# montekki/thaler-study

Hardware: AMD Instinct MI355X
Metric: field mul-adds/sec in sumcheck prover, n=28 vars (higher is better)
Workload: dtype u64

## Files before the change

thaler-study_amd/csrc/engine/abi_context.inc:

```


extern "C" int sc_field_from_modulus(uint64_t p, sc_field* out) {
  if (!out) return SC_ERR_ARG;
  sc::FieldParams fp;
  if (!sc::field_params_from_modulus(p, &fp)) return SC_ERR_ARG;
  out->p = fp.p;
  out->p_inv_neg = fp.p_inv_neg;
  out->r_mod_p = fp.r_mod_p;
  out->r2_mod_p = fp.r2_mod_p;
  return SC_OK;
}

static sc::FieldParams to_params(const sc_field* f) {
  sc::FieldParams fp;
  fp.p = f->p;
  fp.p_inv_neg = f->p_inv_neg;
  fp.r_mod_p = f->r_mod_p;
  fp.r2_mod_p = f->r2_mod_p;
  return fp;
}

extern "C" uint64_t sc_field_to_mont(const sc_field* f, uint64_t canonical) {
  HostField hf(to_params(f));
  return hf.mul(canonical % f->p, f->r2_mod_p);
// ... 70 lines not shown
  SC_CREATE_HIP(hipMemset(ctx->d_wg_tickets, 0, 64 * sizeof(unsigned)));
  SC_CREATE_HIP(hipHostGetDevicePointer((void**)&ctx->d_mailbox, ctx->h_mailbox, 0));
  SC_CREATE_HIP(hipHostMalloc(&ctx->h_tail, kTailSlots * kTailSlotWords * sizeof(u64), hipHostMallocMapped | hipHostMallocCoherent));
  memset(ctx->h_tail, 0, kTailSlots * kTailSlotWords * sizeof(u64));
  SC_CREATE_HIP(hipHostGetDevicePointer((void**)&ctx->d_tail, ctx->h_tail, 0));
  for (int i = kTailSlots - 1; i >= 0; --i) ctx->tail_free.push_back(i);
  SC_CREATE_HIP(hipDeviceSynchronize());
  for (int i = 0; i < sc_ctx::kTimerRing; ++i) {
    SC_CREATE_HIP(hipEventCreate(&ctx->kt_ev[i][0]));
    SC_CREATE_HIP(hipEventCreate(&ctx->kt_ev[i][1]));
  }
#undef SC_CREATE_HIP
  *out = ctx;
  return SC_OK;
}

extern "C" int sc_ctx_destroy(sc_ctx* ctx) {
  if (!ctx) return SC_OK;
  if (is_multi(ctx)) return multi_destroy(ctx);
  (void)hipSetDevice(ctx->device);
  if (ctx->stream) (void)sync_stream(ctx);
  if (ctx->comm && g_rccl.CommDestroy) g_rccl.CommDestroy(ctx->comm);
  for (int q = 0; q < sc::kMaxPeers; ++q)
    if (ctx->peer_ipc_opened[q] && ctx->peer_base[q]) (void)hipIpcCloseMemHandle(ctx->peer_base[q]);
  if (ctx->peer_region) (void)hipFree(ctx->peer_region);
  for (auto& kv : ctx->pool_free) (void)hipFree(kv.second);
  for (auto& kv : ctx->pool_live) (void)hipFree(kv.first);
  if (ctx->d_partials) (void)hipFree(ctx->d_partials);
  if (ctx->d_wg_partials) (void)hipFree(ctx->d_wg_partials);
  if (ctx->d_wg_groups) (void)hipFree(ctx->d_wg_groups);
  if (ctx->d_wg_tickets) (void)hipFree(ctx->d_wg_tickets);
  if (ctx->d_gram_rows) (void)hipFree(ctx->d_gram_rows);
  if (ctx->d_sums) (void)hipFree(ctx->d_sums);
  if (ctx->h_sums) (void)hipHostFree(ctx->h_sums);
  if (ctx->h_mailbox) (void)hipHostFree(ctx->h_mailbox);
  if (ctx->h_tail) (void)hipHostFree(ctx->h_tail);
  if (ctx->h_points) (void)hipHostFree(ctx->h_points);
  if (ctx->d_points) (void)hipFree(ctx->d_points);
  for (u64* tw : ctx->d_rs_twiddles)
    if (tw) (void)hipFree(tw);
  for (u64* tw : ctx->d_rs_twist)
    if (tw) (void)hipFree(tw);
  if (ctx->d_xc_inv) (void)hipFree(ctx->d_xc_inv);
  if (ctx->h_batch_desc) (void)hipHostFree(ctx->h_batch_desc);
  if (ctx->h_batch) (void)hipHostFree(ctx->h_batch);
  if (ctx->d_ticket) (void)hipFree(ctx->d_ticket);
  for (int i = 0; i < sc_ctx::kTimerRing; ++i)
    for (int k = 0; k < 2; ++k)
      if (ctx->kt_ev[i][k]) (void)hipEventDestroy(ctx->kt_ev[i][k]);
  if (ctx->stream) (void)hipStreamDestroy(ctx->stream);
  delete ctx;
  return SC_OK;
}

extern "C" const char* sc_last_error(const sc_ctx* ctx) {
  return ctx ? ctx->err.c_str() : g_create_error.c_str();
}

static int prewarm(sc_ctx* ctx, size_t num_vars);

enum : unsigned { kOptBool = 1, kOptOff = 2, kOptPeer = 4 };
struct OptionSpec {
  const char* name;
  int sc_ctx::*member;
  int64_t lo, hi;
  unsigned flags;
};
const OptionSpec kOptions[] = {
    {"vars_per_pass", &sc_ctx::vars_per_pass, 1, 2, 0},
    {"first_pass_vars", &sc_ctx::first_pass_vars, 0, 4, 0},
    {"grid_pass", &sc_ctx::grid_pass, 0, 1, kOptBool},
    {"grid_log", &sc_ctx::grid_log, 0, 26, 0},
    {"grid_max_vars", &sc_ctx::grid_max_vars, 1, sc::kGridMaxVars, 0},
    {"grid_sharded", &sc_ctx::grid_sharded, 0, 1, kOptBool},
    {"grid_blocks", &sc_ctx::grid_blocks, 0, kWgMaxBlocks, 0},
    {"fold_dma", &sc_ctx::fold_dma, 0, 1, kOptBool},
    {"pipe32", &sc_ctx::pipe32, 0, 1, kOptBool},
    {"pipe32_log", &sc_ctx::pipe32_log, 11, 40, 0},
    {"gram_log", &sc_ctx::gram_log, 14, 40, kOptOff},
    {"wfold_log", &sc_ctx::wfold_log, 12, 40, kOptOff},
    {"wfold_min_log", &sc_ctx::wfold_min_log, 12, 40, 0},
    {"wfold5_min_log", &sc_ctx::wfold5_min_log, 12, 40, 0},
    {"wfold_always", &sc_ctx::wfold_always, 0, 1, kOptBool},
    {"matmul_path", &sc_ctx::matmul_path, 0, 2, 0},
    {"host_tail_log", &sc_ctx::host_tail_log, 0, kTailLogMax, 0},
    {"gp_host_log", &sc_ctx::gp_host_log, 0, sc::kGpHostLogMax, 0},
    {"gp_tree_lv", &sc_ctx::gp_tree_lv, 1, 3, 0},
    {"fr_host_log", &sc_ctx::fr_host_log, 0, sc::kFrHostLogMax, 0},
    {"fr_tree_lv", &sc_ctx::fr_tree_lv, 1, sc::kFrTreeLvMax, 0},
    {"tail_log", &sc_ctx::tail_log, 0, 40, 0},
    {"max_blocks", &sc_ctx::max_blocks, 1, INT64_MAX, 0},
    {"time_kernels", &sc_ctx::time_kernels, 0, 1, kOptBool},
    {"use_mailbox", &sc_ctx::use_mailbox, 0, 1, kOptBool},
    {"nt_load_log", &sc_ctx::nt_load_log, INT64_MIN, INT64_MAX, 0},
    {"nt_store_log", &sc_ctx::nt_store_log, INT64_MIN, INT64_MAX, 0},
    {"pool_contiguous", &sc_ctx::pool_contiguous, 0, 1, kOptBool},
    {"dbg_fold_grab", &sc_ctx::dbg_fold_grab, 0, 16, 0},
    {"rccl_timeout_ms", &sc_ctx::rccl_timeout_ms, 1, 3600000, 0},
    {"arena_log", &sc_ctx::arena_log, 4, 26, kOptPeer},
    {"peer_spin_ms", &sc_ctx::peer_spin_ms, 1, 600000, kOptPeer},
    {"peer_connect_ms", &sc_ctx::peer_connect_ms, 1, 3600000, kOptPeer},
    {"dbg_delay_ms", &sc_ctx::dbg_delay_ms, 0, 10000, kOptPeer},
    {"dbg_skip_tag", &sc_ctx::dbg_skip_tag, 0, 1, kOptBool | kOptPeer},
};
static const OptionSpec* find_option(const char* key) {
  for (const OptionSpec& o : kOptions)
    if (strcmp(o.name, key) == 0) return &o;
  return nullptr;
}

extern "C" int sc_ctx_set_option(sc_ctx* ctx, const char* key, int64_t value) {
  if (!ctx || !key) return SC_ERR_ARG;
  const std::string k(key);
  if (k == "prewarm") return value < 0 ? fail(ctx, SC_ERR_ARG, "prewarm: num_vars must be >= 0") : prewarm(ctx, (size_t)value);
  if (is_multi(ctx)) SC_TRY(multi_set_option(ctx, key, value));
  if (k == "stat_reset") {
    ctx->stat_wait_ns = ctx->stat_launch_ns = 0;
    ctx->pool_peak_words = ctx->pool_live_words;
    return SC_OK;
  }
  const OptionSpec* o = find_option(key);
  if (!o) return fail(ctx, SC_ERR_ARG, "unknown option '%s'", key);
  if (o->member == &sc_ctx::max_blocks && (value < 1 || value > (int64_t)ctx->partial_rows))
    return fail(ctx, SC_ERR_ARG, "max_blocks must be 1..%zu", ctx->partial_rows);
  if (!(o->flags & kOptBool) && (value < o->lo || value > o->hi) && !((o->flags & kOptOff) && value == 0))
    return fail(ctx, SC_ERR_ARG, "%s must be %s%lld..%lld", key, (o->flags & kOptOff) ? "0 (never) or " : "", (long long)o->lo, (long long)o->hi);
  if (o->member == &sc_ctx::arena_log && ctx->peer_region) return fail(ctx, SC_ERR_STATE, "arena_log must be set before sc_ctx_comm_peer_export");
  ctx->*o->member = (o->flags & kOptBool) ? (value ? 1 : 0) : (int)value;
  return SC_OK;
}

static int64_t pool_stat(const sc_ctx* ctx, size_t (*of)(const sc_ctx*)) {
  if (!is_multi(ctx)) return (int64_t)of(ctx);
  int64_t sum = 0;
  for (const sc_ctx* sub : ctx->subs) sum += (int64_t)of(sub);
  return sum;
}

extern "C" int sc_ctx_get_option(const sc_ctx* ctx, const char* key, int64_t* value) {
  if (!ctx || !key || !value) return SC_ERR_ARG;
  const std::string k(key);
  if (k == "stat_wait_ns") *value = (int64_t)(is_multi(ctx) ? ctx->subs[0]->stat_wait_ns : ctx->stat_wait_ns);
  else if (k == "stat_launch_ns") *value = (int64_t)(is_multi(ctx) ? ctx->subs[0]->stat_launch_ns : ctx->stat_launch_ns);
  else if (k == "stat_pool_live_blocks") *value = pool_stat(ctx, [](const sc_ctx* c) { return c->pool_live.size(); });
  else if (k == "stat_pool_live_words") *value = pool_stat(ctx, [](const sc_ctx* c) { return c->pool_live_words; });
  else if (k == "stat_pool_peak_words") *value = pool_stat(ctx, [](const sc_ctx* c) { return c->pool_peak_words; });
  else if (k == "transport") *value = (int64_t)ctx->transport;
  else if (k == "n_devices") *value = is_multi(ctx) ? (int64_t)ctx->subs.size() : 1;
  else if (k == "comm_nranks") {
    int n = ctx->world;
    if (ctx->transport == Transport::kRccl) {
      n = 0;
      if (!g_rccl.CommCount || !ctx->comm || g_rccl.CommCount(ctx->comm, &n) != ncclSuccess)
        return fail(ctx, SC_ERR_RCCL, "ncclCommCount failed");
    }
    *value = n;
  } else if (const OptionSpec* o = find_option(key)) {
    *value = ctx->*o->member;
  } else {
    return fail(ctx, SC_ERR_ARG, "unknown option '%s'", key);
  }
  return SC_OK;
}

extern "C" int sc_ctx_synchronize(sc_ctx* ctx) {
  if (!ctx) return SC_ERR_ARG;
// ... 46 lines not shown
```

thaler-study_amd/csrc/engine/launch.inc:

```

namespace {


#define SC_DISPATCH_FIELD(ctx, F, f, ...)      \
  do {                                         \
    if ((ctx)->gold) {                         \
      typedef sc::GoldilocksMont F;            \
      F f((ctx)->fp);                          \
      __VA_ARGS__;                             \
    } else {                                   \
      typedef sc::MontGeneric F;               \
      F f((ctx)->fp);                          \
      __VA_ARGS__;                             \
    }                                          \
  } while (0)

template <int V>
using IntC = std::integral_constant<int, V>;
template <int... Vs, class Fn>
void with_const(int v, Fn&& fn) {
  (void)((v == Vs && (fn(IntC<Vs>{}), true)) || ...);
}
template <class Fn>
void with_bool(bool b, Fn&& fn) {
// ... 203 lines not shown
    hipLaunchKernelGGL(sc::mailbox_copy_wide_kernel, dim3(1), dim3(sc::kBlock), 0, ctx->stream, (const u64*)ctx->d_sums, 2 * cells,
                       ctx->d_mailbox, wo.seq);
    SC_HIP(ctx, hipGetLastError());
  }
  ctx->mailbox_seq += 1;
  return SC_OK;
}

bool in_tail(const sc_ctx* ctx, const u64* p) { return p && ctx->d_tail && p >= ctx->d_tail && p < ctx->d_tail + kTailSlots * kTailSlotWords; }

int launch_pass(sc_ctx* ctx, int kf, int ks, const u64* A, const u64* B, u64* A2, u64* B2, const u64* r,
                int log_in, bool across_ranks, bool* from_mailbox) {
  if (kf < 0 || kf > 4 || ks < 1 || ks > 3 || (ks == 3 && kf != 0) || (kf == 4 && (ks != 2 || log_in < 12)) || log_in < kf + ks)
    return fail(ctx, SC_ERR_ARG, "launch_pass: kf=%d ks=%d log_in=%d", kf, ks, log_in);
  const sc::FoldW fw = make_weights<sc::FoldW>(ctx, r, kf);
  size_t n_units = (size_t)1 << (log_in - kf - ks);
  const bool pipe32 = kf == 3 && ks == 2 && ctx->pipe32 && n_units % sc::kWave == 0 && log_in >= ctx->pipe32_log;
  const size_t bs = (size_t)sc::pass_block_threads(kf, ks, pipe32 ? 4 : 0);
  int grid = (int)std::min<size_t>(std::max<size_t>((n_units + bs - 1) / bs, 1), (size_t)ctx->max_blocks);
  grid = std::min(grid, pipe32 ? pipe32_resident_blocks(ctx) : pass_resident_blocks(ctx, kf, ks));
  if (kf > 0 && in_tail(ctx, A2) && (grid != 1 || ((size_t)1 << (log_in - kf)) > (size_t)sc::kWave))
    return fail(ctx, SC_ERR_STATE, "launch_pass: a pass_kernel launch of %d blocks would hand 2^%d-entry tables to the host with plain stores", grid,
                log_in - kf);
  const sc::PassOut out = next_pass_out(ctx, across_ranks, challenge_digest(r, kf, ks, log_in), from_mailbox);
  SC_TRY(timer_begin(ctx, SC_KIND_PASS, kf, ks, log_in, (u64)16 << log_in, kf > 0 ? (u64)16 << (log_in - kf) : 0));
  SC_DISPATCH_FIELD(ctx, F, f, launch_pass_t<F>(ctx, f, kf, ks, A, B, A2, B2, fw, n_units, grid, log_in, out, pipe32));
  SC_TRY(commit_pass_out(ctx, out, grid));
  SC_TRY(timer_end(ctx));
  return SC_OK;
}

int wait_mailbox(sc_ctx* ctx, u64 seq);

int check_exchange(sc_ctx* ctx, const char* what) {
  const u64 err = __atomic_load_n(ctx->h_mailbox + sc::kMailboxErr, __ATOMIC_ACQUIRE);
  if (err == 0) return SC_OK;
  if (err & (u64)sc::kXchgTimeout) {
    poison(ctx);
    return fail(ctx, SC_ERR_RCCL, "peer exchange: a rank's %s did not arrive within %d ms (rank %d waited for rank %d at tag %u; that rank's "
                "slot held tag ..%04x)", what, ctx->peer_spin_ms, ctx->rank, (int)((err >> 8) & 0xFF), ctx->xchg_tag, (unsigned)((err >> 16) & 0x3FFF));
  }
  return fail(ctx, SC_ERR_STATE, "the ranks of this sharded prover were given different challenges");
}

int launch_grid_pass(sc_ctx* ctx, int kf, int ks, const u64* A, const u64* B, u64* A2, u64* B2, const u64* r, int log_in, bool across_ranks) {
  if (kf < 0 || kf > sc::kGridMaxVars || ks < 1 || ks > sc::kGridMaxVars || log_in < kf + ks)
    return fail(ctx, SC_ERR_ARG, "launch_grid_pass: kf=%d ks=%d log_in=%d", kf, ks, log_in);
  if (!ctx->use_mailbox) return fail(ctx, SC_ERR_STATE, "launch_grid_pass needs the host mailbox");
  const sc::GridW gw = make_weights<sc::GridW>(ctx, r, kf);
  const size_t n_out = (size_t)1 << (log_in - kf);
  const int resident = std::min(resident_grid(ctx, ctx->gold ? kernel_ptr(&sc::wgrid_pass_kernel<sc::GoldilocksMont, 5, false>)
                                                             : kernel_ptr(&sc::wgrid_pass_kernel<sc::MontGeneric, 5, false>),
                                              sc::kBlock, 2 * ctx->num_cus),
                                kWgMaxBlocks);
  constexpr size_t kWaves = sc::kBlock / sc::kWave;
  const size_t n_iter = (n_out + sc::kWgEntries - 1) / sc::kWgEntries;
  const size_t cap = ctx->grid_blocks > 0 ? (size_t)std::min(ctx->grid_blocks, resident) : (size_t)resident;
  const int grid = (int)std::max<size_t>(1, std::min<size_t>((n_iter + kWaves - 1) / kWaves, cap));
  const sc::WgOut wo = next_wide_out(ctx, across_ranks, challenge_digest(r, kf, ks, log_in), true, in_tail(ctx, A2));
  SC_TRY(timer_begin(ctx, SC_KIND_GRID_PASS, kf, ks, log_in, (u64)16 << log_in, kf > 0 ? (u64)16 << (log_in - kf) : 0));
  const bool pf = (kf == 0 || kf == 2) && n_iter > (size_t)grid * kWaves;
  SC_DISPATCH_FIELD(ctx, F, f, with_bool(pf, [&](auto PF) {
    with_const<1, 2, 3, 4, 5>(ks, [&](auto KS) {
      hipLaunchKernelGGL((sc::wgrid_pass_kernel<F, KS, PF>), dim3(grid), dim3(sc::kBlock), 0, ctx->stream, f, A, B, A2, B2, gw, kf, n_out, wo);
    });
  }));
  return commit_wide_out(ctx, wo, pow3(ks));
}
bool wfold_has(int kf, int ks) { return (kf == 4 && ks == 5) || (kf == 5 && ks >= 3 && ks <= 5); }
int wfold_resident_blocks(sc_ctx* ctx) {
  const void* fn = ctx->gold ? kernel_ptr(&sc::wfold_pass_kernel<sc::GoldilocksMont, 4, 5, true>)
                             : kernel_ptr(&sc::wfold_pass_kernel<sc::MontGeneric, 4, 5, true>);
  return std::min(resident_grid(ctx, fn, sc::kWfThreads, ctx->num_cus), kWgMaxBlocks);
}
int launch_wfold_pass(sc_ctx* ctx, int kf, int ks, const u64* A, const u64* B, u64* A2, u64* B2, const u64* r, int log_in, bool across_ranks) {
  if (log_in < 12 || !A2 || !B2 || !wfold_has(kf, ks)) return fail(ctx, SC_ERR_ARG, "launch_wfold_pass: kf=%d ks=%d log_in=%d", kf, ks, log_in);
  if (!ctx->use_mailbox) return fail(ctx, SC_ERR_STATE, "launch_wfold_pass needs the host mailbox");
  const sc::FoldW fw = make_weights<sc::FoldW>(ctx, r, 4);
  const u64 r_top = kf == 5 ? r[4] : 0;
  const size_t n_tiles = (size_t)1 << (log_in - 12);
  const int grid = (int)std::max<size_t>(1, std::min<size_t>(std::min<size_t>(n_tiles, (size_t)wfold_resident_blocks(ctx)), (size_t)ctx->max_blocks));
  const sc::WgOut wo = next_wide_out(ctx, across_ranks, challenge_digest(r, kf, ks, log_in) ^ 0x77666f6cu, true, false);
  SC_TRY(timer_begin(ctx, SC_KIND_WFOLD_PASS, kf, ks, log_in, (u64)16 << log_in, (u64)16 << (log_in - kf)));
  SC_DISPATCH_FIELD(ctx, F, f, with_bool(log_in >= ctx->nt_load_log, [&](auto NT) {
    auto go = [&](auto KF, auto KS) {
      hipLaunchKernelGGL((sc::wfold_pass_kernel<F, KF, KS, NT>), dim3(grid), dim3(sc::kWfThreads), 0, ctx->stream, f, A, B, A2, B2, fw, r_top, n_tiles, wo);
    };
    if (kf == 4) go(IntC<4>{}, IntC<5>{});
    else with_const<3, 4, 5>(ks, [&](auto KS) { go(IntC<5>{}, KS); });
  }));
  return commit_wide_out(ctx, wo, pow3(ks));
}

constexpr int kGramK = 4;
constexpr int kGramMaxBlocks = 1024;
int gram_workspace(sc_ctx* ctx) {
  if (ctx->d_gram_rows) return SC_OK;
  const size_t bytes = (size_t)kGramMaxBlocks * sc::kGramRowWords * sizeof(u64) + 64;
  u64* p = nullptr;
  SC_HIP(ctx, hipMalloc(&p, bytes));
  hipError_t e = hipMemsetAsync(p, 0, bytes, ctx->stream);
  const int lds = sc::kGramStages * sc::kGramStageBytes;
  const void* fns[4] = {reinterpret_cast<const void*>(&sc::gram_pass_kernel<sc::GoldilocksMont, kGramK, true>),
                        reinterpret_cast<const void*>(&sc::gram_pass_kernel<sc::GoldilocksMont, kGramK, false>),
                        reinterpret_cast<const void*>(&sc::gram_pass_kernel<sc::MontGeneric, kGramK, true>),
                        reinterpret_cast<const void*>(&sc::gram_pass_kernel<sc::MontGeneric, kGramK, false>)};
  for (int i = 0; i < 4 && e == hipSuccess; ++i) e = hipFuncSetAttribute(fns[i], hipFuncAttributeMaxDynamicSharedMemorySize, lds);
  if (e != hipSuccess) {
    (void)hipFree(p);
    SC_HIP(ctx, e);
  }
  ctx->d_gram_rows = p;
  return SC_OK;
}
int launch_gram_pass(sc_ctx* ctx, const u64* A, const u64* B, int log_in, bool across_ranks) {
  typedef sc::GramGeo<kGramK> G;
  if (!ctx->use_mailbox) return fail(ctx, SC_ERR_STATE, "launch_gram_pass needs the host mailbox");
  const size_t len = (size_t)1 << log_in;
  if (len < (size_t)G::kEntriesPerStep * sc::kGramStages) return fail(ctx, SC_ERR_ARG, "launch_gram_pass: 2^%d entries are too few", log_in);
  const size_t n_steps = len / G::kEntriesPerStep;
  size_t blocks = 1;
  while (blocks * 2 <= (size_t)std::min(std::min(ctx->num_cus, ctx->max_blocks), kGramMaxBlocks)) blocks *= 2;
  size_t n_partials = std::min(blocks, n_steps / sc::kGramStages);
  while (n_steps / n_partials > (size_t)G::kMaxSteps) n_partials *= 2;
  const size_t spp = n_steps / n_partials;
  const int grid = (int)std::min(blocks, n_partials);
  SC_TRY(gram_workspace(ctx));
  const sc::WgOut wo = next_wide_out(ctx, across_ranks, challenge_digest(nullptr, 0, kGramK, log_in) ^ 0x6772616du, false, false);
  unsigned* ticket = reinterpret_cast<unsigned*>(ctx->d_gram_rows + (size_t)kGramMaxBlocks * sc::kGramRowWords);
  SC_TRY(timer_begin(ctx, SC_KIND_GRAM_PASS, 0, kGramK, log_in, (u64)16 << log_in, (u64)grid * sc::kGramRowWords * sizeof(u64)));
  const unsigned char* a8 = reinterpret_cast<const unsigned char*>(A);
  const unsigned char* b8 = reinterpret_cast<const unsigned char*>(B);
  const int lds = sc::kGramStages * sc::kGramStageBytes;
  SC_DISPATCH_FIELD(ctx, F, f, with_bool(log_in >= ctx->nt_load_log, [&](auto NT) {
    hipLaunchKernelGGL((sc::gram_pass_kernel<F, kGramK, NT>), dim3(grid), dim3(sc::kGramThreads), lds, ctx->stream, f, a8, b8,
                       (unsigned)n_partials, (unsigned)spp, ctx->d_gram_rows, ticket, wo);
  }));
  return commit_wide_out(ctx, wo, pow3(kGramK));
}

int collect_grid(sc_ctx* ctx, int ks, bool across_ranks, u64* out) {
  SC_TRY(wait_mailbox(ctx, ctx->mailbox_seq));
  const int cells = pow3(ks);
  const u64* wide = ctx->h_mailbox + sc::kMailboxWide;
  if (!across_ranks) {
    for (int c = 0; c < cells; ++c) out[c] = wide[c];
    return SC_OK;
  }
  HostField hf(ctx->fp);
  if (ctx->transport == Transport::kHost) {
    std::vector<u64> limbs(2 * (size_t)cells);
    for (int c = 0; c < cells; ++c) {
      limbs[2 * c] = wide[c] & 0xFFFFFFFFull;
      limbs[2 * c + 1] = wide[c] >> 32;
    }
    if (ctx->host_allreduce(ctx->host_user, limbs.data(), limbs.size()) != 0)
      return fail(ctx, SC_ERR_RCCL, "host all-reduce callback failed");
    for (int c = 0; c < cells; ++c) out[c] = hf.recombine(limbs[2 * c], limbs[2 * c + 1]);
    return SC_OK;
  }
  if (ctx->transport == Transport::kPeer) SC_TRY(check_exchange(ctx, "sums"));
  for (int c = 0; c < cells; ++c) out[c] = hf.recombine(wide[2 * c], wide[2 * c + 1]);
  return SC_OK;
}

int rank_pass(sc_ctx* ctx, int kf, const u64* A, const u64* B, u64* A2, u64* B2, const u64* r, u64* out) {
  if (ctx->transport != Transport::kPeer || !ctx->use_mailbox || kf < 0 || kf > sc::kGridMaxVars || ctx->log_world < 1 || ctx->log_world > 3)
    return fail(ctx, SC_ERR_STATE, "rank_pass: needs the peer transport, the mailbox and 2..8 ranks");
  const sc::GridW gw = make_weights<sc::GridW>(ctx, r, kf);
  const sc::WgOut wo = next_wide_out(ctx, true, challenge_digest(r, kf, ctx->log_world, kf) ^ 0x72616e6bu, true, false);
  SC_TRY(timer_begin(ctx, SC_KIND_GRID_PASS, kf, ctx->log_world, kf, (u64)16 << kf, (u64)16 << ctx->log_world));
  SC_DISPATCH_FIELD(ctx, F, f,
// ... 10 lines not shown
```

thaler-study_amd/csrc/kernels/grid_pass.hpp:

```cpp
#pragma once

namespace sc {

constexpr int kGridChunk = 256;
constexpr int kGridMaxVars = 5;
constexpr int kGridMaxCells = 243;
constexpr int kMailboxWide = 64;
constexpr int kMailboxWords = kMailboxWide + 512;
constexpr int kWgEntries = 32;
constexpr int kWgGroupBlocks = 32;
struct GridW {
  u64 w[1 << kGridMaxVars];
};
struct WgOut {
  u64* partials;
  u64* group_rows;
  unsigned* tickets;
  u64* mailbox;
  u64 seq;
  u64* limbs_dev;
  PeerX px;
  int host_out = 0;
};
template <class F, int KF>
// ... 279 lines not shown
    return;
  }
  if (tid < CELLS) __hip_atomic_store(out.mailbox + kMailboxWide + tid, total, __ATOMIC_RELAXED, __HIP_MEMORY_SCOPE_SYSTEM);
  asm volatile("s_waitcnt vmcnt(0)" ::: "memory");
  __syncthreads();
  if (tid == 0) __hip_atomic_store(out.mailbox + kMailboxSeq, out.seq, __ATOMIC_RELEASE, __HIP_MEMORY_SCOPE_SYSTEM);
}

template <class F, int KS>
__device__ __forceinline__ void wgrid_finish(const F& f, u64 total, const WgOut& out) {
  constexpr int kPow3[6] = {1, 3, 9, 27, 81, 243};
  constexpr int cells = kPow3[KS];
  __shared__ int lds_flag;
  const int tid = threadIdx.x;
  if (gridDim.x > 1) {
    const int n_blocks = gridDim.x, group = blockIdx.x / kWgGroupBlocks, n_groups = (n_blocks + kWgGroupBlocks - 1) / kWgGroupBlocks;
    const int group_size = min(kWgGroupBlocks, n_blocks - group * kWgGroupBlocks);
    if (tid < cells)
      __hip_atomic_store(out.partials + (size_t)blockIdx.x * kGridChunk + tid, total, __ATOMIC_RELAXED, __HIP_MEMORY_SCOPE_AGENT);
    asm volatile("s_waitcnt vmcnt(0)" ::: "memory");
    __syncthreads();
    if (tid == 0) {
      const unsigned t = __hip_atomic_fetch_add(out.tickets + 1 + group, 1u, __ATOMIC_RELAXED, __HIP_MEMORY_SCOPE_AGENT);
      const int last = (t == (unsigned)group_size - 1) ? 1 : 0;
      if (last) {
        __builtin_amdgcn_fence(__ATOMIC_ACQUIRE, "agent");
        asm volatile("s_waitcnt vmcnt(0)" ::: "memory");
      }
      lds_flag = last;
    }
    __syncthreads();
    if (!lds_flag) return;
    total = 0;
    if (tid < cells) {
      u64 x[kWgGroupBlocks];
#pragma unroll
      for (int q = 0; q < kWgGroupBlocks; ++q)
        x[q] = (q < group_size) ? __hip_atomic_load(out.partials + (size_t)(group * kWgGroupBlocks + q) * kGridChunk + tid, __ATOMIC_RELAXED,
                                                    __HIP_MEMORY_SCOPE_AGENT)
                                : 0;
#pragma unroll
      for (int q = 0; q < kWgGroupBlocks; ++q) total = f.add(total, x[q]);
    }
    if (n_groups > 1) {
      __syncthreads();
      if (tid < cells)
        __hip_atomic_store(out.group_rows + (size_t)group * kGridChunk + tid, total, __ATOMIC_RELAXED, __HIP_MEMORY_SCOPE_AGENT);
      asm volatile("s_waitcnt vmcnt(0)" ::: "memory");
      __syncthreads();
      if (tid == 0) {
        const unsigned t = __hip_atomic_fetch_add(out.tickets, 1u, __ATOMIC_RELAXED, __HIP_MEMORY_SCOPE_AGENT);
        const int last = (t == (unsigned)n_groups - 1) ? 1 : 0;
        if (last) {
          __builtin_amdgcn_fence(__ATOMIC_ACQUIRE, "agent");
          asm volatile("s_waitcnt vmcnt(0)" ::: "memory");
        }
        lds_flag = last;
      }
      __syncthreads();
      if (!lds_flag) return;
      total = 0;
      if (tid < cells) {
        u64 x[kWgGroupBlocks];
#pragma unroll
        for (int q = 0; q < kWgGroupBlocks; ++q)
          x[q] = (q < n_groups) ? __hip_atomic_load(out.group_rows + (size_t)q * kGridChunk + tid, __ATOMIC_RELAXED, __HIP_MEMORY_SCOPE_AGENT) : 0;
#pragma unroll
        for (int q = 0; q < kWgGroupBlocks; ++q) total = f.add(total, x[q]);
      }
    }
    if (tid <= n_groups) __hip_atomic_store(out.tickets + tid, 0u, __ATOMIC_RELAXED, __HIP_MEMORY_SCOPE_AGENT);
  }
  publish_cells<cells>(out, total);
}

template <class F, int KS, bool PF>
__global__ void __launch_bounds__(kBlock)
wgrid_pass_kernel(F f, const u64* __restrict__ A, const u64* __restrict__ B, u64* __restrict__ A2, u64* __restrict__ B2,
                  GridW gw, int kf, size_t n_out, WgOut out) {
  const u64 total = wgrid_body<F, KS, PF>(f, A, B, A2, B2, gw, kf, n_out, out.host_out != 0);
  wgrid_finish<F, KS>(f, total, out);
}

constexpr int kWfThreads = 512;
template <class F, int KF, int KS, bool NT>
__global__ void __launch_bounds__(kWfThreads)
wfold_pass_kernel(F f, const u64* __restrict__ A, const u64* __restrict__ B, u64* __restrict__ A2, u64* __restrict__ B2, FoldW fw,
                  u64 r_top, size_t n_tiles, WgOut out) {
  static_assert(KF == 4 || KF == 5, "four or five pending challenges");
  static_assert(KS >= 1 && KS <= 5, "one to five rounds");
  constexpr int OUT = 4, NPS = 8, NP = 32;
  constexpr int OUTS = kWave >> (KF - 4);
  constexpr int TILE_OUT = OUT * OUTS;
  constexpr int NPO = TILE_OUT / (2 * kWave);
  constexpr int kWaves = kWfThreads / kWave;
  constexpr int kPow3[6] = {1, 3, 9, 27, 81, 243};
  constexpr int cells = kPow3[KS], G = 1 << KS, gpi = kWgEntries >> KS, pairs = gpi * cells;
  constexpr int kRegionWords = 1024 + 512 + 512;
  __shared__ u64 lds_all[kWaves * kRegionWords];
  __shared__ int cell_of[kWgEntries], suffix_of[kWgEntries];
  __shared__ unsigned lds_next;
  typedef __attribute__((address_space(3))) u64 lds_u64;
  const int tid = threadIdx.x, lane = tid & (kWave - 1), wave = tid / kWave;
  if (tid < kWgEntries) {
    int c = 0, u = 0, p3 = 1;
    for (int m = 0; m < KS; ++m) {
      c += ((tid >> (KS - 1 - m)) & 1) * p3;
      u += ((tid >> m) & 1) * p3;
      p3 *= 3;
    }
    cell_of[tid] = c;
    suffix_of[tid] = u;
  }
  if (tid == 0) lds_next = 0;
  __syncthreads();
  ull2* const reg = reinterpret_cast<ull2*>(lds_all + (size_t)wave * kRegionWords);
  u64* const xchg = lds_all + (size_t)wave * kRegionWords + 1024;
  u64* const ef = xchg + 512;
  const int tbl = lane >> 5, ent = lane & (kWgEntries - 1);
  const int slot = tbl * kGridChunk + (ent >> KS) * cells + cell_of[ent & (G - 1)];
  unsigned step[KS][3];
#pragma clang loop unroll(full)
  for (int j = 0; j < KS; ++j) {
    const int low = KS - 1 - j, pj = kPow3[j], stride = kPow3[low], items = (gpi * pj) << low;
    const unsigned inv = (1u << 20) / (unsigned)pj + 1u;
#pragma clang loop unroll(full)
    for (int q = 0; q < 3; ++q) {
      const int idx = lane + kWave * q;
      unsigned d = 0;
      if (idx < 2 * items) {
        const int tb = idx >= items ? 1 : 0, id = idx - tb * items;
        const int sfx = id & ((1 << low) - 1), t = id >> low;
        const int g = (int)(((unsigned)t * inv) >> 20), pp = t - g * pj;
        d = 0x80000000u | (unsigned)(size_t)(lds_u64*)(ef + tb * kGridChunk + g * cells + pp * 3 * stride + suffix_of[sfx]);
      }
      step[j][q] = d;
    }
  }
  typename F::Acc acc[4];
#pragma unroll
  for (int k = 0; k < 4; ++k) f.acc_zero(acc[k]);

  const ull2* __restrict__ Ap = reinterpret_cast<const ull2*>(A);
  const ull2* __restrict__ Bp = reinterpret_cast<const ull2*>(B);
  ull2* __restrict__ A2p = reinterpret_cast<ull2*>(A2);
  ull2* __restrict__ B2p = reinterpret_cast<ull2*>(B2);
  const int rot = wave & 3;
  auto next_tile = [&]() -> size_t {
    unsigned c = 0;
    if (lane == 0) c = __hip_atomic_fetch_add(&lds_next, 1u, __ATOMIC_RELAXED, __HIP_MEMORY_SCOPE_WORKGROUP);
    return (size_t)__builtin_amdgcn_readfirstlane(c) * gridDim.x + blockIdx.x;
  };
  auto load_sub = [&](const ull2* __restrict__ T, size_t tile, int o, ull2 (&p)[NPS]) {
    const ull2* src = T + tile * kWave * NP + (size_t)o * NPS * kWave + lane;
#pragma unroll
    for (int k = 0; k < NPS; ++k) p[k] = ld16<NT>(src + k * kWave);
  };
  auto stash = [&](const ull2 (&p)[NPS]) {
#pragma unroll
    for (int k = 0; k < NPS; ++k) reg[swz_slot<NPS>(64 * k + lane)] = p[k];
  };
  auto fold16 = [&]() -> u64 {
    typename F::Acc3 sacc;
    f.acc3_zero(sacc);
#pragma unroll
    for (int m = 0; m < NPS; ++m) {
      const ull2 x = reg[swz_slot<NPS>(NPS * lane + m)];
      f.acc3_mac(sacc, x.x, fw.w[2 * m]);
      f.acc3_mac(sacc, x.y, fw.w[2 * m + 1]);
    }
    const u64 h = f.acc3_get(sacc);
    if constexpr (KF == 5) {
      const u64 hn = __shfl_xor(h, 1);
      return f.add(h, f.mul(r_top, f.sub(hn, h)));
    } else {
      return h;
    }
  };
  auto put = [&](u64* dst, int o, u64 x) {
    if constexpr (KF == 5) {
      if ((lane & 1) == 0) dst[OUTS * o + (lane >> 1)] = x;
    } else {
      dst[OUTS * o + lane] = x;
    }
  };
  auto grid_group = [&](int grp) {
    ef[slot] = xchg[kWave * OUT * tbl + kWgEntries * grp + ent];
    wave_lds_sync();
#pragma clang loop unroll(full)
    for (int j = 0; j < KS; ++j) {
      const int st = kPow3[KS - 1 - j];
#pragma clang loop unroll(full)
      for (int q = 0; q < 3; ++q) {
        if (2 * ((gpi * kPow3[j]) << (KS - 1 - j)) > kWave * q) {
          const unsigned d = step[j][q];
          if (d != 0) {
            lds_u64* const x = (lds_u64*)(size_t)(d & 0x7FFFFFFFu);
            x[2 * st] = f.sub(x[st], x[0]);
          }
        }
      }
      wave_lds_sync();
    }
#pragma unroll
    for (int k = 0; k < 4; ++k) {
      const int p = lane + kWave * k;
      if (p < pairs) f.acc_mac(acc[k], ef[p], ef[kGridChunk + p]);
    }
    wave_lds_sync();
  };
  ull2 pa[NPS], pb[NPS];
  size_t tile = next_tile();
  if (tile < n_tiles) {
    load_sub(Ap, tile, rot, pa);
    load_sub(Bp, tile, rot, pb);
  }
  while (tile < n_tiles) {
    const size_t next = next_tile();
#pragma unroll
    for (int i = 0; i < OUT; ++i) {
      const int o = (i + rot) & 3, no = (i + 1 + rot) & 3;
      stash(pa);
      wave_lds_sync();
      if (i + 1 < OUT) load_sub(Ap, tile, no, pa);
      else if (next < n_tiles) load_sub(Ap, next, no, pa);
      const u64 xa = fold16();
      wave_lds_sync();
      stash(pb);
      wave_lds_sync();
      if (i + 1 < OUT) load_sub(Bp, tile, no, pb);
      else if (next < n_tiles) load_sub(Bp, next, no, pb);
      const u64 xb = fold16();
      put(xchg, o, xa);
      put(xchg + kWave * OUT, o, xb);
      wave_lds_sync();
#pragma unroll 1
      for (int g = 0; g < OUTS / kWgEntries; ++g) grid_group(o * (OUTS / kWgEntries) + g);
    }
    {
      const ull2* xo = reinterpret_cast<const ull2*>(xchg);
      const size_t o0 = tile * kWave * NPO;
#pragma unroll
      for (int k = 0; k < NPO; ++k) {
        const size_t q = o0 + (size_t)k * kWave + lane;
        st16<false>(A2p + q, xo[kWave * k + lane]);
        st16<false>(B2p + q, xo[kWave * OUT / 2 + kWave * k + lane]);
      }
    }
    wave_lds_sync();
    if (wave == 0 && blockIdx.x < 8) asm volatile("buffer_wbl2 sc1" ::: "memory");
    tile = next;
  }
  __syncthreads();
  u64* const red = lds_all;
#pragma unroll
  for (int k = 0; k < 4; ++k) {
    const int p = lane + kWave * k;
    red[wave * kGridChunk + p] = (p < pairs) ? f.acc_get(acc[k]) : 0;
  }
  __syncthreads();
  u64 total = 0;
  if (tid < cells) {
    for (int w = 0; w < kWaves; ++w)
      for (int g = 0; g < gpi; ++g) total = f.add(total, red[w * kGridChunk + g * cells + tid]);
  }
  wgrid_finish<F, KS>(f, total, out);
}

template <class F>
__global__ void __launch_bounds__(kBlock)
rank_pass_kernel(F f, const u64* __restrict__ A, const u64* __restrict__ B, u64* __restrict__ A2, u64* __restrict__ B2, GridW gw, int kf,
                 WgOut out) {
  const PeerX& px = out.px;
  __shared__ u64 ta[kMaxPeers], tb[kMaxPeers];
  __shared__ int worst;
  const int tid = threadIdx.x;
  const size_t par = (size_t)(px.tag & 1u) * kMaxPeers * kInboxWords;
  int err = 0;
  if (tid == 0) worst = 0;
  if (tid < 2) {
    const u64* __restrict__ src = tid ? B : A;
    const int fan = 1 << kf;
    u64 v = 0;
    for (int c = 0; c < fan; ++c) v = f.add(v, f.mul(src[c], gw.w[c]));
    const ull2 pair = {((u64)px.tag << 32) | (v & 0xFFFFFFFFull), ((u64)px.tag << 32) | (v >> 32)};
    const size_t mine = par + (size_t)px.rank * kInboxWords + kInboxWide + 2 * (size_t)tid;
    for (int q = 0; q < px.world; ++q) st16_system(px.inbox[q] + mine, pair);
  }
  if (tid == 2) {
    const u64 g = ((u64)px.tag << 32) | (u64)px.digest;
    for (int q = 0; q < px.world; ++q)
      __hip_atomic_store(px.inbox[q] + par + (size_t)px.rank * kInboxWords + kInboxDigest, g, __ATOMIC_RELAXED, __HIP_MEMORY_SCOPE_SYSTEM);
  }
  const unsigned long long t0 = wall_clock64();
  if (tid < 3 * px.world) {
    const int r = tid / 3, what = tid % 3;
    const u64* base = px.inbox[px.rank] + par + (size_t)r * kInboxWords;
    unsigned spins = 0;
    while (true) {
      if (what < 2) {
        const ull2 g = ld16_system(base + kInboxWide + 2 * what);
        if ((unsigned)(g.x >> 32) == px.tag && (unsigned)(g.y >> 32) == px.tag) {
          const u64 v = (g.x & 0xFFFFFFFFull) | (g.y << 32);
          (what ? tb : ta)[r] = v;
          break;
        }
      } else {
        const u64 g = __hip_atomic_load(base + kInboxDigest, __ATOMIC_RELAXED, __HIP_MEMORY_SCOPE_SYSTEM);
        if ((unsigned)(g >> 32) == px.tag) {
          err = ((unsigned)g != px.digest) ? kXchgDigest : 0;
          break;
        }
      }
      if ((++spins & 31) == 0 && wall_clock64() - t0 > px.spin_ticks) {
        err = kXchgTimeout | (r << 8);
        break;
      }
      __builtin_amdgcn_s_sleep(1);
    }
  }
  __syncthreads();
  if (err) atomicMax(&worst, err);
  __syncthreads();
  if (worst == 0) {
    if (tid < px.world) {
      A2[tid] = ta[tid];
      B2[tid] = tb[tid];
    }
    int g = 0;
    while ((1 << g) < px.world) ++g;
    int cells = 1;
    for (int j = 0; j < g; ++j) cells *= 3;
    if (tid < cells) {
      int d[3] = {0, 0, 0};
// ... 34 lines not shown
```

thaler-study_amd/csrc/sumcheck_hip.hip:

```cpp
#include <dlfcn.h>
#include <hip/hip_runtime.h>
#include <rccl/rccl.h>

#include <algorithm>
#include <chrono>
#include <cstdarg>
#include <cstdio>
#include <cstring>
#include <atomic>
#include <condition_variable>
#include <functional>
#include <map>
#include <memory>
#include <mutex>
#include <new>
#include <set>
#include <string>
#include <thread>
#include <type_traits>
#include <vector>

#include "../../include/sumcheck_hip.h"
#include "kernels.hpp"

// ... 19 lines not shown

RcclApi g_rccl;
std::string g_create_error;

bool load_rccl(std::string* why) {
  if (g_rccl.handle) return true;
  const char* chosen = getenv("SC_RCCL_LIBRARY");
  const char* names[] = {"librccl.so.1", "librccl.so", "/opt/rocm/lib/librccl.so.1"};
  void* h = nullptr;
  if (chosen && *chosen) {
    h = dlopen(chosen, RTLD_NOW | RTLD_LOCAL);
    if (!h) {
      *why = std::string("dlopen(SC_RCCL_LIBRARY=") + chosen + ") failed: " + dlerror();
      return false;
    }
  } else {
    for (const char* n : names) {
      h = dlopen(n, RTLD_NOW | RTLD_LOCAL);
      if (h) break;
    }
  }
  if (!h) {
    *why = std::string("dlopen(librccl) failed: ") + dlerror();
    return false;
  }
  RcclApi a;
  a.handle = h;
  a.GetUniqueId = (decltype(a.GetUniqueId))dlsym(h, "ncclGetUniqueId");
  a.CommInitRank = (decltype(a.CommInitRank))dlsym(h, "ncclCommInitRank");
  a.CommDestroy = (decltype(a.CommDestroy))dlsym(h, "ncclCommDestroy");
  a.CommCount = (decltype(a.CommCount))dlsym(h, "ncclCommCount");
  a.AllReduce = (decltype(a.AllReduce))dlsym(h, "ncclAllReduce");
  a.AllGather = (decltype(a.AllGather))dlsym(h, "ncclAllGather");
  a.GetErrorString = (decltype(a.GetErrorString))dlsym(h, "ncclGetErrorString");
  a.CommAbort = (decltype(a.CommAbort))dlsym(h, "ncclCommAbort");
  a.CommGetAsyncError = (decltype(a.CommGetAsyncError))dlsym(h, "ncclCommGetAsyncError");
  if (!a.GetUniqueId || !a.CommInitRank || !a.CommDestroy || !a.AllReduce || !a.AllGather) {
    *why = "librccl is missing a required symbol";
    return false;
  }
  g_rccl = a;
  return true;
}

enum class Transport { kNone, kRccl, kHost, kPeer, kLocal };
constexpr int kMaxSubs = 8;
constexpr int kTailLogMax = 12;
constexpr int kTailSoftLog = 11;
constexpr int kTailEntries = 1 << kTailLogMax;
constexpr int kTailSmallLog = 5;
constexpr int kTailSlots = 32;
constexpr size_t kTailSlotWords = 2 * (size_t)kTailEntries;
constexpr int kWgMaxBlocks = 1024;

}

struct sc_ctx {
  sc::FieldParams fp;
  bool gold = false;
  int device = 0;
  hipStream_t stream = nullptr;
  mutable std::string err;
  mutable bool poisoned = false;

  int vars_per_pass = 2;
  int first_pass_vars = 0;
  int grid_pass = 1;
  int grid_log = 20;
  int grid_max_vars = 5;
  int grid_sharded = 1;
  int grid_blocks = 0;
  u64* d_wg_partials = nullptr;
  u64* d_wg_groups = nullptr;
  unsigned* d_wg_tickets = nullptr;
  u64* d_gram_rows = nullptr;
  int fold_dma = 1;
  int pipe32 = 1, pipe32_log = 20;
  int gram_log = 21;
  int host_tail_log = kTailLogMax;
  int wfold_log = 40;
  int wfold_min_log = 21;
  int wfold5_min_log = 24;
  int wfold_always = 0;
  int matmul_path = 0;
  int gp_host_log = 10;
  int gp_tree_lv = sc::kGpTreeLv;
  int fr_host_log = 9;
  int fr_tree_lv = sc::kFrTreeLv;
  int tail_log = 16;
  int max_blocks = 768;
  int num_cus = 256;
  std::map<const void*, int> resident_grid;
  int time_kernels = 0;
  uint64_t stat_wait_ns = 0, stat_launch_ns = 0;
  int nt_load_log = 22;
  int nt_store_log = 25;

  u64* d_partials = nullptr;
  u64* d_sums = nullptr;
  u64* h_sums = nullptr;
  size_t partial_rows = 0;
  unsigned* d_ticket = nullptr;
  bool fold_lds_allowed[4][2] = {};
  unsigned ticket_base = 0;
  u64* h_mailbox = nullptr;
  u64* d_mailbox = nullptr;
  u64 mailbox_seq = 0;
  int use_mailbox = 1;

  std::multimap<size_t, u64*> pool_free;
  std::map<u64*, size_t> pool_live;
  size_t pool_live_words = 0, pool_peak_words = 0;

  Transport transport = Transport::kNone;
  int rank = 0, world = 1, log_world = 0;
  ncclComm_t comm = nullptr;
  sc_allreduce_fn host_allreduce = nullptr;
  sc_allgather_fn host_allgather = nullptr;
  void* host_user = nullptr;
  u64* peer_region = nullptr;
  size_t peer_region_words = 0;
  bool peer_exported = false;
  u64* peer_base[sc::kMaxPeers] = {};
  bool peer_ipc_opened[sc::kMaxPeers] = {};
  int arena_log = 17;
  unsigned xchg_tag = 0;
  unsigned xchg_next = 0;
  unsigned gather_count = 0;
  int peer_spin_ms = 2000;
  int rccl_timeout_ms = 30000;
  mutable bool comm_failed = false;
  int peer_connect_ms = 120000;
  int dbg_delay_ms = 0;
  int dbg_skip_tag = 0;
  int dbg_fold_grab = 0;
  int pool_contiguous = 0;

  std::vector<sc_ctx*> subs;
  sc_ctx* parent = nullptr;
  struct MultiRuntime* mrt = nullptr;
  u64* h_tail = nullptr;
  u64* d_tail = nullptr;
  std::vector<int> tail_free;
  u64* h_points = nullptr;
  u64* d_points = nullptr;
  void* h_batch_desc = nullptr;
  size_t batch_desc_bytes = 0;
  u64* h_batch = nullptr;
  u64* d_batch = nullptr;
  size_t batch_words = 0;
  bool rs_root_known = false;
  int rs_two_adicity = 0;
  u64 rs_w_max = 0;
  u64* d_rs_twiddles[15] = {};
  u64* d_rs_twist[25] = {};
  std::set<const void*> lds_allowed;
  u64* d_xc_inv = nullptr;

  static constexpr int kTimerRing = 64;
  static constexpr size_t kLaunchLogCap = 1 << 16;
  hipEvent_t kt_ev[kTimerRing][2] = {};
  sc_launch_record kt_meta[kTimerRing] = {};
  int kt_used = 0;
  double kt_ms = 0.0;
  long kt_n = 0;
  std::vector<sc_launch_record> launch_log;
// ... 303 lines not shown
```

Baseline: 871.7 billion.

## Batch wfold output stores into wall-clock time slots with deferred held tiles

Adds a time-slotted store scheme to the wfold pass kernel. Each wave holds its folded output tile in registers and writes it back only during periodic wall-clock windows, and the L2 writeback flush is issued once per slot instead of once per tile. The aim is to group write traffic into bursts so it interferes less with the streaming loads. This is on by default for kf=4 with log_in>=25, at the cost of extra registers for the held tile, clock reads and LDS state.

```diff
diff --git a/thaler-study_amd/csrc/engine/abi_context.inc b/thaler-study_amd/csrc/engine/abi_context.inc
--- a/thaler-study_amd/csrc/engine/abi_context.inc
+++ b/thaler-study_amd/csrc/engine/abi_context.inc
@@ -176,6 +176,9 @@
     {"wfold_min_log", &sc_ctx::wfold_min_log, 12, 40, 0},
     {"wfold5_min_log", &sc_ctx::wfold5_min_log, 12, 40, 0},
     {"wfold_always", &sc_ctx::wfold_always, 0, 1, kOptBool},
+    {"wfold_slot_period", &sc_ctx::wfold_slot_period, -1, 1 << 24, 0},
+    {"wfold_slot_width", &sc_ctx::wfold_slot_width, 0, 1 << 24, 0},
+    {"wfold_slot_stagger", &sc_ctx::wfold_slot_stagger, 0, 1, kOptBool},
     {"matmul_path", &sc_ctx::matmul_path, 0, 2, 0},
     {"host_tail_log", &sc_ctx::host_tail_log, 0, kTailLogMax, 0},
     {"gp_host_log", &sc_ctx::gp_host_log, 0, sc::kGpHostLogMax, 0},
diff --git a/thaler-study_amd/csrc/engine/launch.inc b/thaler-study_amd/csrc/engine/launch.inc
--- a/thaler-study_amd/csrc/engine/launch.inc
+++ b/thaler-study_amd/csrc/engine/launch.inc
@@ -309,12 +309,24 @@
   const int grid = (int)std::max<size_t>(1, std::min<size_t>(std::min<size_t>(n_tiles, (size_t)wfold_resident_blocks(ctx)), (size_t)ctx->max_blocks));
   const sc::WgOut wo = next_wide_out(ctx, across_ranks, challenge_digest(r, kf, ks, log_in) ^ 0x77666f6cu, true, false);
   SC_TRY(timer_begin(ctx, SC_KIND_WFOLD_PASS, kf, ks, log_in, (u64)16 << log_in, (u64)16 << (log_in - kf)));
+  sc::WfSlots sl;
+  if (ctx->wfold_slot_period < 0) {
+    sl.period = (kf == 4 && log_in >= 25) ? 2400u : 0u;
+    sl.width = 600u;
+  } else {
+    sl.period = (unsigned)ctx->wfold_slot_period;
+    sl.width = (unsigned)ctx->wfold_slot_width;
+    sl.stagger = (unsigned)ctx->wfold_slot_stagger;
+  }
   SC_DISPATCH_FIELD(ctx, F, f, with_bool(log_in >= ctx->nt_load_log, [&](auto NT) {
-    auto go = [&](auto KF, auto KS) {
-      hipLaunchKernelGGL((sc::wfold_pass_kernel<F, KF, KS, NT>), dim3(grid), dim3(sc::kWfThreads), 0, ctx->stream, f, A, B, A2, B2, fw, r_top, n_tiles, wo);
-    };
-    if (kf == 4) go(IntC<4>{}, IntC<5>{});
-    else with_const<3, 4, 5>(ks, [&](auto KS) { go(IntC<5>{}, KS); });
+    with_bool(sl.period != 0, [&](auto SLOTS) {
+      auto go = [&](auto KF, auto KS) {
+        hipLaunchKernelGGL((sc::wfold_pass_kernel<F, KF, KS, NT, SLOTS>), dim3(grid), dim3(sc::kWfThreads), 0, ctx->stream, f, A, B, A2, B2, fw, r_top,
+                           n_tiles, wo, sl);
+      };
+      if (kf == 4) go(IntC<4>{}, IntC<5>{});
+      else with_const<3, 4, 5>(ks, [&](auto KS) { go(IntC<5>{}, KS); });
+    });
   }));
   return commit_wide_out(ctx, wo, pow3(ks));
 }
diff --git a/thaler-study_amd/csrc/kernels/grid_pass.hpp b/thaler-study_amd/csrc/kernels/grid_pass.hpp
--- a/thaler-study_amd/csrc/kernels/grid_pass.hpp
+++ b/thaler-study_amd/csrc/kernels/grid_pass.hpp
@@ -385,11 +385,17 @@
   wgrid_finish<F, KS>(f, total, out);
 }
 
+#define SC_WFOLD_SLOTS 1
+struct WfSlots {
+  unsigned period = 0;
+  unsigned width = 0;
+  unsigned stagger = 0;
+};
 constexpr int kWfThreads = 512;
-template <class F, int KF, int KS, bool NT>
+template <class F, int KF, int KS, bool NT, bool SLOTS = false>
 __global__ void __launch_bounds__(kWfThreads)
 wfold_pass_kernel(F f, const u64* __restrict__ A, const u64* __restrict__ B, u64* __restrict__ A2, u64* __restrict__ B2, FoldW fw,
-                  u64 r_top, size_t n_tiles, WgOut out) {
+                  u64 r_top, size_t n_tiles, WgOut out, WfSlots sl) {
   static_assert(KF == 4 || KF == 5, "four or five pending challenges");
   static_assert(KS >= 1 && KS <= 5, "one to five rounds");
   constexpr int OUT = 4, NPS = 8, NP = 32;
@@ -403,8 +409,25 @@
   __shared__ u64 lds_all[kWaves * kRegionWords];
   __shared__ int cell_of[kWgEntries], suffix_of[kWgEntries];
   __shared__ unsigned lds_next;
+  constexpr unsigned kNoTile = ~0u;
+  __shared__ unsigned lds_slots[4];
+  __shared__ unsigned lds_wave[kWaves][2];
   typedef __attribute__((address_space(3))) u64 lds_u64;
   const int tid = threadIdx.x, lane = tid & (kWave - 1), wave = tid / kWave;
+  auto lds_word = [](const unsigned* p) -> unsigned {
+    return (unsigned)__builtin_amdgcn_readfirstlane((int)*(const volatile unsigned*)p);
+  };
+  if constexpr (SLOTS) {
+    if (tid == 0) {
+      lds_slots[0] = sl.period;
+      lds_slots[1] = sl.width;
+      lds_slots[2] = sl.stagger ? (blockIdx.x & 7u) * (sl.period >> 3) : 0u;
+    }
+    if (lane == 0) {
+      lds_wave[wave][0] = kNoTile;
+      lds_wave[wave][1] = ((unsigned)wall_clock64() + (sl.stagger ? (blockIdx.x & 7u) * (sl.period >> 3) : 0u) - sl.width) / sl.period;
+    }
+  }
   if (tid < kWgEntries) {
     int c = 0, u = 0, p3 = 1;
     for (int m = 0; m < KS; ++m) {
@@ -512,6 +535,16 @@
     }
     wave_lds_sync();
   };
+  ull2 held[2 * NPO];
+  auto store_held = [&](unsigned t) {
+#pragma unroll
+    for (int k = 0; k < NPO; ++k) {
+      const size_t q = (size_t)t * kWave * NPO + (size_t)k * kWave + lane;
+      st16<false>(A2p + q, held[2 * k]);
+      st16<false>(B2p + q, held[2 * k + 1]);
+    }
+    lds_wave[wave][0] = kNoTile;
+  };
   ull2 pa[NPS], pb[NPS];
   size_t tile = next_tile();
   if (tile < n_tiles) {
@@ -523,6 +556,17 @@
 #pragma unroll
     for (int i = 0; i < OUT; ++i) {
       const int o = (i + rot) & 3, no = (i + 1 + rot) & 3;
+      if constexpr (SLOTS) {
+        const unsigned period = lds_word(&lds_slots[0]), width = lds_word(&lds_slots[1]);
+        const unsigned t = (unsigned)wall_clock64() + lds_word(&lds_slots[2]);
+        const unsigned ht = lds_word(&lds_wave[wave][0]);
+        if (ht != kNoTile && t % period < width) store_held(ht);
+        if (wave == 0 && blockIdx.x < 8) {
+          const unsigned k = (t - width) / period;
+          if (k != lds_word(&lds_wave[0][1])) asm volatile("buffer_wbl2 sc1" ::: "memory");
+          lds_wave[0][1] = k;
+        }
+      }
       stash(pa);
       wave_lds_sync();
       if (i + 1 < OUT) load_sub(Ap, tile, no, pa);
@@ -543,16 +587,33 @@
     {
       const ull2* xo = reinterpret_cast<const ull2*>(xchg);
       const size_t o0 = tile * kWave * NPO;
-#pragma unroll
-      for (int k = 0; k < NPO; ++k) {
-        const size_t q = o0 + (size_t)k * kWave + lane;
-        st16<false>(A2p + q, xo[kWave * k + lane]);
-        st16<false>(B2p + q, xo[kWave * OUT / 2 + kWave * k + lane]);
+      if (SLOTS && lds_word(&lds_slots[1]) != 0) {
+        const unsigned ht = lds_word(&lds_wave[wave][0]);
+        if (ht != kNoTile) store_held(ht);
+#pragma unroll
+        for (int k = 0; k < NPO; ++k) {
+          held[2 * k] = xo[kWave * k + lane];
+          held[2 * k + 1] = xo[kWave * OUT / 2 + kWave * k + lane];
+        }
+        lds_wave[wave][0] = (unsigned)tile;
+      } else {
+#pragma unroll
+        for (int k = 0; k < NPO; ++k) {
+          const size_t q = o0 + (size_t)k * kWave + lane;
+          st16<false>(A2p + q, xo[kWave * k + lane]);
+          st16<false>(B2p + q, xo[kWave * OUT / 2 + kWave * k + lane]);
+        }
       }
     }
     wave_lds_sync();
-    if (wave == 0 && blockIdx.x < 8) asm volatile("buffer_wbl2 sc1" ::: "memory");
+    if constexpr (!SLOTS) {
+      if (wave == 0 && blockIdx.x < 8) asm volatile("buffer_wbl2 sc1" ::: "memory");
+    }
     tile = next;
+  }
+  if constexpr (SLOTS) {
+    const unsigned ht = lds_word(&lds_wave[wave][0]);
+    if (ht != kNoTile) store_held(ht);
   }
   __syncthreads();
   u64* const red = lds_all;
diff --git a/thaler-study_amd/csrc/sumcheck_hip.hip b/thaler-study_amd/csrc/sumcheck_hip.hip
--- a/thaler-study_amd/csrc/sumcheck_hip.hip
+++ b/thaler-study_amd/csrc/sumcheck_hip.hip
@@ -125,6 +125,7 @@
   int wfold_min_log = 21;
   int wfold5_min_log = 24;
   int wfold_always = 0;
+  int wfold_slot_period = -1, wfold_slot_width = 0, wfold_slot_stagger = 0;
   int matmul_path = 0;
   int gp_host_log = 10;
   int gp_tree_lv = sc::kGpTreeLv;
```

Measured after the change: 903.3 billion (median of 6 runs). 3.6% higher.
